# bwittmann/transoar

Hardware: AMD Instinct MI355X
Metric: training-step CT volumes/s, 160x160x256 Focused-Decoder (higher is better)
Workload: dtype bf16

## Files before the change

### include/transoar_conv3d.h

```cpp
#ifndef TRANSOAR_CONV3D_H
#define TRANSOAR_CONV3D_H

#include <stddef.h>
#include <stdint.h>

#ifdef __cplusplus
extern "C" {
#endif

enum {
  TRANSOAR_CONV_OK = 0,
  TRANSOAR_CONV_ERR_NULL = -1,
  TRANSOAR_CONV_ERR_DIM = -2,
  TRANSOAR_CONV_ERR_CHANNELS = -3
};

int transoar_conv3d_k3_forward(const void* x, const void* wk, const float* bias, void* y,
                               int N, int D, int H, int W, int Cin, int Cout, int stride,
                               int dilated_input, void* hip_stream);

int transoar_conv3d_k3_wgrad(const void* gyT, const void* xT3, float* dw, int N, int D, int H,
                             int W, int Cin, int Do, int Ho, int Wo, int Cout, int stride_dh,
                             void* hip_stream);

int transoar_conv3d_k3_forward_c1(const void* x, const void* wk, const float* bias, void* y, int N, int D, int H,
                                  int W, int Cout, void* hip_stream);

int transoar_conv3d_k3_stat_rows(int N, int D, int H, int W, int Cin, int Cout, int stride);
int transoar_conv3d_k3_forward_stats(const void* x, const void* wk, const float* bias, void* y, float* stat_part,
                                     int N, int D, int H, int W, int Cin, int Cout, void* hip_stream);

int transoar_conv3d_c1_forward(const void* x, const float* w, void* y, int N, int D, int H,
                               int W, int Cout, void* hip_stream);

int transoar_conv3d_k3_wgrad_lds(const void* x, const void* dy, float* partial, int n_wg, int N, int D,
                                 int H, int W, int Cin, int Cout, int ci0, int ci_n, int co0, int co_n,
                                 void* hip_stream);
int transoar_conv3d_k3_wgrad_tr(const void* x, const void* dy, float* partial, int n_wg, int N, int D,
                                 int H, int W, int Cin, int Cout, int ci0, int ci_n, int co0, int co_n,
                                 void* hip_stream);

int transoar_conv3d_c1_wgrad(const void* x, const void* dy, float* partial, int n_partial, int N, int D,
                             int H, int W, int Cout, void* hip_stream);
int transoar_conv3d_c1_wgrad_tr(const void* x, const void* dy, float* partial, int n_partial, int N, int D,
                                int H, int W, int Cout, void* hip_stream);

int transoar_layout_bf16(const void* in, void* out, int N, long V, int C, int to_channels_first,
                         void* hip_stream);

int transoar_conv3d_abi_version(void);

#ifdef __cplusplus
}
#endif
#endif
```

### include/transoar_instnorm.h

```cpp
#ifndef TRANSOAR_INSTNORM_H
#define TRANSOAR_INSTNORM_H

#ifdef __cplusplus
extern "C" {
#endif

enum {
  TRANSOAR_IN_OK = 0,
  TRANSOAR_IN_ERR_NULL = -1,
  TRANSOAR_IN_ERR_DIM = -2,
  TRANSOAR_IN_ERR_CHANNELS = -3
};

int transoar_instnorm_relu_forward(const void* x, const float* gamma, const float* beta, void* y,
                                   double* stats_ws, float* mean_rstd, int N, long V, int C,
                                   float eps, int relu, void* hip_stream);

int transoar_instnorm_relu_forward_parts(const void* x, const float* gamma, const float* beta, void* y,
                                         const float* stat_part, int rows_per_sample, double* stats_ws,
                                         float* mean_rstd, int N, long V, int C, float eps, int relu,
                                         void* hip_stream);

int transoar_instnorm_relu_backward(const void* x, const void* dy, const float* gamma,
                                    const float* beta, const float* mean_rstd, void* dx,
                                    double* red_ws, float* dparams, int N, long V, int C, int relu,
                                    void* hip_stream);

int transoar_instnorm_abi_version(void);

#ifdef __cplusplus
}
#endif
#endif
```

### transoar_amd/backbone.py

```python
import os

import torch
from torch import nn

from . import instnorm
from .conv3d import Conv3dK3, to_ncdhw
from .position_encoding import PositionEmbeddingLearned3D, PositionEmbeddingSine3D
from .swin_encoder import ConvPatchMerging, EncoderSwinBlock, PatchMerging
from .refine_block import DecoderDefAttnBlock
from .token_linear import token_linear


class EncoderCnnBlock(nn.Module):

    def __init__(self, in_channels, out_channels, kernel_size, stride, padding=1, bias=False,
                 affine=True, eps=1e-05):
        super().__init__()
        kernel_size, stride = tuple(kernel_size), tuple(stride)
        self._block = nn.Sequential(
            Conv3dK3(in_channels, out_channels, kernel_size, stride=stride, padding=padding, bias=bias),
            nn.InstanceNorm3d(out_channels, affine=affine, eps=eps),
            nn.ReLU(inplace=True),
            Conv3dK3(out_channels, out_channels, kernel_size, stride=1, padding=padding, bias=bias),
            nn.InstanceNorm3d(out_channels, affine=affine, eps=eps),
            nn.ReLU(inplace=True),
        )
        self._affine = affine

    fused_norm = True

    def _norm_relu(self, x, norm, part=None):
        if (EncoderCnnBlock.fused_norm and self._affine and x.dtype == torch.bfloat16
                and instnorm.supported(x, norm.num_features)):
            return instnorm.instance_norm_relu(x, norm.weight, norm.bias, norm.eps, relu=True, part=part)
        return torch.relu_(norm(x))

    def _conv_norm_relu(self, conv, norm, x):
        if (EncoderCnnBlock.fused_norm and self._affine and isinstance(conv, Conv3dK3) and norm.num_features <= 32):
            y, part = conv.forward_with_stats(x)
            if part is not None and not (y.dtype == torch.bfloat16 and instnorm.supported(y, norm.num_features)):
                part = None
            return self._norm_relu(y, norm, part)
        return self._norm_relu(conv(x), norm)

    def forward(self, x):
        if not x.is_cuda:
            return self._block(x)
        blk = self._block
        x = self._conv_norm_relu(blk[0], blk[1], x)
        return self._conv_norm_relu(blk[3], blk[4], x)


class Encoder(nn.Module):
    def __init__(self, config, debug=False):
        super().__init__()
        self._debug = debug
        self._stages = nn.ModuleList()
        cin, cout = config["in_channels"], config["start_channels"]
        swin = bool(config["use_encoder_attn"])
        depths = list(config["depths"])
        dpr = [float(v) for v in torch.linspace(0, config["drop_path_rate"], sum(depths))]
        merge = ConvPatchMerging if config["conv_merging"] else PatchMerging
        for stage_id, (kernel, stride) in enumerate(zip(config["conv_kernels"], config["strides"])):
            if swin and stage_id > 1:
                k = stage_id - 2
                stage = EncoderSwinBlock(
                    dim=cin, depth=depths[k], num_heads=config["num_heads"][k], window_size=config["window_size"],
                    mlp_ratio=config["mlp_ratio"], qkv_bias=config["qkv_bias"], qk_scale=config["qk_scale"],
                    drop=config["drop_rate"], attn_drop=config["attn_drop_rate"],
                    drop_path=dpr[sum(depths[:k]):sum(depths[:k + 1])], downsample=merge)
            else:
                stage = EncoderCnnBlock(cin, cout, kernel, stride)
            self._stages.append(stage)
            cin, cout = cout, cout * 2

    def forward(self, x):
        outputs = {}
        for i, stage in enumerate(self._stages):
            x = stage(x)
            outputs["C%d" % i] = x
        if self._debug:
            print("AttnFPN encoder shapes:", {k: list(v.shape) for k, v in outputs.items()})
            self._debug = False
        return outputs


def _gemm_conv_ok(f):
    return (f.is_cuda and f.dtype == torch.bfloat16 and f.dim() == 5 and f.shape[1] % 8 == 0
            and f.is_contiguous(memory_format=torch.channels_last_3d)
            and torch.is_autocast_enabled() and torch.get_autocast_gpu_dtype() == torch.bfloat16)
# ... 116 lines not shown
```

### transoar_amd/conv3d.py

```python
import ctypes
import os

import torch
import torch.nn.functional as F
from torch import nn

from . import _native
from . import rows as _rows
from . import conv_gemm as _cg

_PKG = os.path.dirname(os.path.abspath(__file__))
_LIB_PATH = os.path.join(_PKG, "libtransoar_conv3d.so")
ABI_VERSION = 5


def _load():
    if not os.path.exists(_LIB_PATH):
        raise _native.NativeLibraryError("%s is not built (python transoar_amd/_build.py)" % _LIB_PATH)
    lib = ctypes.CDLL(_LIB_PATH)
    i, p = ctypes.c_int, ctypes.c_void_p
    lib.transoar_conv3d_k3_forward.restype = i
    lib.transoar_conv3d_k3_forward.argtypes = [p, p, p, p] + [i] * 8 + [p]
    lib.transoar_conv3d_k3_wgrad.restype = i
    lib.transoar_conv3d_k3_wgrad.argtypes = [p, p, p] + [i] * 10 + [p]
    lib.transoar_conv3d_k3_wgrad_lds.restype = i
    lib.transoar_conv3d_k3_wgrad_lds.argtypes = [p, p, p, i] + [i] * 10 + [p]
    lib.transoar_conv3d_k3_wgrad_tr.restype = i
    lib.transoar_conv3d_k3_wgrad_tr.argtypes = [p, p, p, i] + [i] * 10 + [p]
    lib.transoar_conv3d_c1_wgrad.restype = i
    lib.transoar_conv3d_c1_wgrad.argtypes = [p, p, p, i] + [i] * 5 + [p]
    lib.transoar_conv3d_c1_wgrad_tr.restype = i
    lib.transoar_conv3d_c1_wgrad_tr.argtypes = [p, p, p, i] + [i] * 5 + [p]
    lib.transoar_conv3d_k3_stat_rows.restype = i
    lib.transoar_conv3d_k3_stat_rows.argtypes = [i] * 7
    lib.transoar_conv3d_k3_forward_stats.restype = i
    lib.transoar_conv3d_k3_forward_stats.argtypes = [p, p, p, p, p] + [i] * 6 + [p]
    lib.transoar_conv3d_k3_forward_c1.restype = i
    lib.transoar_conv3d_k3_forward_c1.argtypes = [p, p, p, p] + [i] * 5 + [p]
    lib.transoar_conv3d_c1_forward.restype = i
    lib.transoar_conv3d_c1_forward.argtypes = [p, p, p] + [i] * 5 + [p]
    lib.transoar_layout_bf16.restype = i
    lib.transoar_layout_bf16.argtypes = [p, p, i, ctypes.c_long, i, i, p]
    lib.transoar_conv3d_abi_version.restype = i
    if lib.transoar_conv3d_abi_version() != ABI_VERSION:
        raise _native.NativeLibraryError("%s: ABI mismatch, rebuild" % _LIB_PATH)
    return lib


lib = _load()
CL3D = torch.channels_last_3d


def _check(rc, what):
    if rc != 0:
        raise RuntimeError("%s failed with code %d" % (what, rc))


def _stream():
    return torch.cuda.current_stream().cuda_stream


class _Relayout(torch.autograd.Function):

    @staticmethod
    def forward(ctx, t, to_channels_first):
        return _relayout_raw(t, to_channels_first)

    @staticmethod
    def backward(ctx, g):
        return g, None


def _relayout(t, to_channels_first):
    if t.requires_grad and torch.is_grad_enabled():
        return _Relayout.apply(t, to_channels_first)
    return _relayout_raw(t, to_channels_first)


def _relayout_raw(t, to_channels_first):
    n, c = t.shape[:2]
    v = t.shape[2] * t.shape[3] * t.shape[4]
    out = torch.empty(t.shape, dtype=t.dtype, device=t.device,
                      memory_format=torch.contiguous_format if to_channels_first else CL3D)
    with torch.cuda.device(t.device):
        _check(lib.transoar_layout_bf16(t.data_ptr(), out.data_ptr(), n, v, c, 1 if to_channels_first else 0,
# ... 59 lines not shown
        return None
    if ci == 1:
        y = torch.empty((n, d, h, w, co), dtype=torch.bfloat16, device=x.device).permute(0, 4, 1, 2, 3)
    else:
        y = torch.empty((n, co, d, h, w), dtype=torch.bfloat16, device=x.device, memory_format=CL3D)
    part = torch.empty((rows, 2, 32), dtype=torch.float32, device=x.device)
    with torch.cuda.device(x.device):
        _check(lib.transoar_conv3d_k3_forward_stats(x.data_ptr(), wk.data_ptr(), bias.data_ptr() if bias is not None else None,
                                                    y.data_ptr(), part.data_ptr(), n, d, h, w, ci, co, _stream()),
               "transoar_conv3d_k3_forward_stats")
    return y, part


def wgrad_operands(x, gy, stride):
    ow = gy.shape[4]
    gy_t = gy.permute(1, 0, 2, 3, 4).contiguous()
    x_t = F.pad(x.permute(1, 0, 2, 3, 4).contiguous(), (1, 1))
    x_t3 = torch.stack([x_t[..., kw: kw + stride * (ow - 1) + 1: stride] for kw in range(3)])
    return x_t3, gy_t


def conv3d_k3_wgrad(x, gy, stride):
    n, ci, d, h, w = x.shape
    co, od, oh, ow = gy.shape[1], gy.shape[2], gy.shape[3], gy.shape[4]
    x_t3, gy_t = wgrad_operands(x, gy, stride)
    cin_p = (ci + 7) // 8 * 8
    dw = torch.zeros((27, co, cin_p), dtype=torch.float32, device=x.device)
    with torch.cuda.device(x.device):
        _check(lib.transoar_conv3d_k3_wgrad(gy_t.data_ptr(), x_t3.data_ptr(), dw.data_ptr(), n, d, h, ow, ci,
                                            od, oh, ow, co, stride, _stream()), "transoar_conv3d_k3_wgrad")
    return dw[:, :, :ci].view(3, 3, 3, co, ci).permute(3, 4, 0, 1, 2)


C1_WGRAD_PARTIALS = 3200
C1_WGRAD_TR = os.environ.get("TRANSOAR_C1_WGRAD_TR", "1") != "0"
C1_WGRAD_TR_PARTIALS = 1024


def _colsum(partial):
    flat = partial.view(partial.shape[0], -1)
    return _rows.colsum_small(flat) if _rows.colsum_small_usable(flat) else flat.sum(0)


def conv3d_c1_wgrad(x, gy):
    n, _, d, h, w = x.shape
    co = gy.shape[1]
    tr = C1_WGRAD_TR and co % 8 == 0 and w % 64 == 0 and w <= 256
    n_part = min(C1_WGRAD_TR_PARTIALS, n * d * h) if tr else min(C1_WGRAD_PARTIALS, max(1, (n * d * h + 3) // 4))
    partial = torch.empty((n_part, 32, 32), dtype=torch.float32, device=x.device)
    with torch.cuda.device(x.device):
        fn = lib.transoar_conv3d_c1_wgrad_tr if tr else lib.transoar_conv3d_c1_wgrad
        _check(fn(x.data_ptr(), gy.data_ptr(), partial.data_ptr(), n_part, n, d, h, w, co, _stream()), "transoar_conv3d_c1_wgrad")
    return _colsum(partial).view(32, 32)[:co, :27].reshape(co, 1, 3, 3, 3)


LDS_WGRAD_GROUPS = 512
LDS_WGRAD_TR = os.environ.get("TRANSOAR_WGRAD_TR", "1") != "0"
LDS_WGRAD_TR_GROUPS = 512


def conv3d_k3_wgrad_lds(x, gy):
    n, ci, d, h, w = x.shape
    co = gy.shape[1]
    dw = torch.empty((co, ci, 27), dtype=torch.float32, device=x.device)
    for co0 in range(0, co, 32):
        for ci0 in range(0, ci, 32):
            co_n, ci_n = min(32, co - co0), min(32, ci - ci0)
            groups = LDS_WGRAD_TR_GROUPS if LDS_WGRAD_TR else LDS_WGRAD_GROUPS
            fn = lib.transoar_conv3d_k3_wgrad_tr if LDS_WGRAD_TR else lib.transoar_conv3d_k3_wgrad_lds
            partial = torch.empty((groups, 27, 32, 32), dtype=torch.float32, device=x.device)
            with torch.cuda.device(x.device):
                _check(fn(x.data_ptr(), gy.data_ptr(), partial.data_ptr(), groups, n, d, h, w, ci, co, ci0, ci_n, co0, co_n, _stream()),
                       "transoar_conv3d_k3_wgrad_lds")
            dw[co0:co0 + co_n, ci0:ci0 + ci_n] = _colsum(partial).view(27, 32, 32)[:, :co_n, :ci_n].permute(1, 2, 0)
    return dw.view(co, ci, 3, 3, 3)


def lds_wgrad_supported(x, gy):
    ci, co = x.shape[1], gy.shape[1]
    return (ci % 8 == 0 and co % 8 == 0 and ci <= 64 and co <= 64 and x.shape[-1] % 64 == 0
            and x.is_contiguous(memory_format=CL3D) and gy.is_contiguous(memory_format=CL3D))


def c1_wgrad_supported(x, gy):
    return x.shape[1] == 1 and gy.shape[1] <= 32 and x.shape[-1] % 16 == 0 and x.is_contiguous()


class _Conv3dK3(torch.autograd.Function):
    @staticmethod
    def forward(ctx, x, weight, bias, stride, packs=None, want_stats=False):
        xb = x.to(torch.bfloat16).contiguous() if x.shape[1] == 1 else _as_ndhwc(x)
        ci = xb.shape[1]
        wkt = None
        if want_stats:
            res = None
            if stride == 1 and (ci == 1 or not _use_gemm(ci, weight.shape[0], stride)):
                wk = _pack_taps(F.pad(weight, (0, 0, 0, 0, 0, 0, 0, 7)) if ci == 1 else weight)
                res = conv3d_k3_forward_stats(xb, wk, bias.float() if bias is not None else None)
            if res is not None:
                ctx.save_for_backward(xb, weight, None)
                ctx.stride, ctx.has_bias, ctx.two = stride, bias is not None, True
                ctx.mark_non_differentiable(res[1])
                return res
        ctx.two = want_stats
        if ci == 1:
            n, _, d, h, w = xb.shape
# ... 96 lines not shown
```

### transoar_amd/csrc/conv3d.hip

```cpp
#include <hip/hip_runtime.h>
#include <algorithm>
#include <cstdlib>
#include <stdint.h>

#include "../../include/transoar_conv3d.h"

namespace transoar {

using bf16x8 = __attribute__((ext_vector_type(8))) __bf16;
using f32x16 = __attribute__((ext_vector_type(16))) float;
using u32x4c = __attribute__((ext_vector_type(4))) unsigned int;
using u32x2c = __attribute__((ext_vector_type(2))) unsigned int;

__device__ __forceinline__ unsigned short f2bf(float f) {
  return __builtin_bit_cast(unsigned short, static_cast<__bf16>(f));
}
__device__ __forceinline__ unsigned pack2_bf16(float a, float b) {
  typedef float f32x2_t __attribute__((ext_vector_type(2)));
  typedef __bf16 bf16x2_t __attribute__((ext_vector_type(2)));
  return __builtin_bit_cast(unsigned, __builtin_convertvector(f32x2_t{a, b}, bf16x2_t));
}
__device__ __forceinline__ float bf2f(unsigned short b) {
  return __uint_as_float(static_cast<unsigned int>(b) << 16);
}
// ... 168 lines not shown
  __shared__ __attribute__((aligned(16))) unsigned char halo[kLtHaloVox * VP];
  const int lane = threadIdx.x & 63;
  const int wave = threadIdx.x >> 6;
  const int col = lane & 31, half = lane >> 5;

  const long per = (n_tiles + 7) >> 3;
  const long trow = static_cast<long>(blockIdx.x & 7) * per + (blockIdx.x >> 3);
  if (trow >= n_tiles || (blockIdx.x >> 3) >= per) return;
  const int th = static_cast<int>(trow % tiles_h);
  const long t2 = trow / tiles_h;
  const int td = static_cast<int>(t2 % tiles_d);
  const int n = static_cast<int>(t2 / tiles_d);
  const int d0 = td * kLtD, h0 = th * kLtH;

  const __amdgpu_buffer_rsrc_t xr =
      __builtin_amdgcn_make_buffer_rsrc(const_cast<unsigned short*>(x), 0, static_cast<int>(x_bytes), 0x00020000);
  const __amdgpu_buffer_rsrc_t wr =
      __builtin_amdgcn_make_buffer_rsrc(const_cast<unsigned short*>(wk), 0, static_cast<int>(w_bytes), 0x00020000);

  constexpr int PIECES = kLtHaloVox * CPT;
  constexpr int ROUNDS = (PIECES + 255) / 256;
  u32x4c stage[ROUNDS];
  auto fetch = [&](int w0) {
#pragma unroll
    for (int r = 0; r < ROUNDS; ++r) {
      const int p = r * 256 + static_cast<int>(threadIdx.x);
      const int hv = p / CPT, c = p - hv * CPT;
      const int row = hv / (kLtW + 2), wi = hv - row * (kLtW + 2);
      const int hd = row / (kLtH + 2), hh = row - hd * (kLtH + 2);
      const int d = d0 - 1 + hd, h = h0 - 1 + hh, w = w0 - 1 + wi;
      const bool ok = p < PIECES && static_cast<unsigned>(d) < static_cast<unsigned>(g.D) &&
                      static_cast<unsigned>(h) < static_cast<unsigned>(g.H) && static_cast<unsigned>(w) < static_cast<unsigned>(g.W);
      if constexpr (C1) {
        const unsigned off = ok ? static_cast<unsigned>(((n * g.D + d) * g.H + h) * g.W + w) * 2u : kOOB;
        const unsigned short v = __builtin_amdgcn_raw_buffer_load_b16(xr, off, 0, 0);
        stage[r] = u32x4c{static_cast<unsigned>(v), 0u, 0u, 0u};
      } else {
        const unsigned off = ok ? (static_cast<unsigned>(((n * g.D + d) * g.H + h) * g.W + w) * CPT + c) * 16u : kOOB;
        stage[r] = __builtin_amdgcn_raw_buffer_load_b128(xr, off, 0, 0);
      }
    }
  };
  float srun[4] = {0.f, 0.f, 0.f, 0.f};
  fetch(0);
  for (int tw = 0; tw < tiles_w; ++tw) {
  const int w0 = tw * kLtW;
#pragma unroll
  for (int r = 0; r < ROUNDS; ++r) {
    const int p = r * 256 + static_cast<int>(threadIdx.x);
    if (p < PIECES) *reinterpret_cast<u32x4c*>(halo + p * 16) = stage[r];
  }
  __syncthreads();
  if (tw + 1 < tiles_w) fetch(w0 + kLtW);

  f32x16 acc[MT];
#pragma unroll
  for (int t = 0; t < MT; ++t)
#pragma unroll
    for (int r = 0; r < 16; ++r) acc[t][r] = 0.f;

  constexpr int n_chunks = 9 * CPT;
  constexpr int n_steps = (n_chunks + 1) / 2;
  const unsigned char* lane_base = halo + ((wave * (kLtH + 2)) * (kLtW + 2) + col) * VP;
  const unsigned w_lane = static_cast<unsigned>(col) * g.CinP * 2u;
  const bool co_ok = col < g.Cout;
  const unsigned w_tap = static_cast<unsigned>(g.Cout) * g.CinP * 2u;
  if constexpr (CPT == 3 && !C1) {
    auto load_w = [&](auto gc, int kd, bf16x8 (&wf)[3]) {
      constexpr int gi = decltype(gc)::value;
      constexpr int kw0 = gi < 3 ? gi : (gi == 3 ? 0 : 2), kw1 = gi < 3 ? gi : (gi == 3 ? 1 : 2);
      constexpr int c80 = gi < 3 ? 0 : 2, c81 = gi < 3 ? 1 : 2;
      const bool ok = co_ok && (half ? gi != 4 : true);
      const unsigned base = kd * 9 * w_tap + w_lane + (half ? kw1 * w_tap + c81 * 16 : kw0 * w_tap + c80 * 16);
#pragma unroll
      for (int kh = 0; kh < 3; ++kh)
        wf[kh] = __builtin_bit_cast(bf16x8, __builtin_amdgcn_raw_buffer_load_b128(wr, ok ? base + kh * 3 * w_tap : kOOB, 0, 0));
    };
    bf16x8 wcur[3];
    load_w(ConvIntC<0>{}, 0, wcur);
#pragma unroll 1
    for (int kd = 0; kd < 3; ++kd) {
      const unsigned char* plane = lane_base + kd * (kLtH + 2) * (kLtW + 2) * VP;
      static_for_conv<0, 5>([&](auto gc) {
        constexpr int gi = decltype(gc)::value;
        constexpr int kw0 = gi < 3 ? gi : (gi == 3 ? 0 : 2), kw1 = gi < 3 ? gi : (gi == 3 ? 1 : 2);
        constexpr int c80 = gi < 3 ? 0 : 2, c81 = gi < 3 ? 1 : 2;
        bf16x8 wnext[3];
        if constexpr (gi + 1 < 5) load_w(ConvIntC<gi + 1>{}, kd, wnext);
        else load_w(ConvIntC<0>{}, kd + 1, wnext);
        const unsigned char* src = plane + (half ? kw1 * VP + c81 * 16 : kw0 * VP + c80 * 16);
        bf16x8 xr[MT + 2];
#pragma unroll
        for (int r = 0; r < MT + 2; ++r) xr[r] = __builtin_bit_cast(bf16x8, *reinterpret_cast<const u32x4c*>(src + r * (kLtW + 2) * VP));
#pragma unroll
        for (int kh = 0; kh < 3; ++kh)
#pragma unroll
          for (int t = 0; t < MT; ++t) acc[t] = __builtin_amdgcn_mfma_f32_32x32x16_bf16(wcur[kh], xr[t + kh], acc[t], 0, 0, 0);
#pragma unroll
        for (int kh = 0; kh < 3; ++kh) wcur[kh] = wnext[kh];
      });
    }
  } else {
#pragma unroll 1
  for (int kd = 0; kd < 3; ++kd) {
    const unsigned char* plane = lane_base + kd * (kLtH + 2) * (kLtW + 2) * VP;
    const unsigned w_plane = kd * 9 * w_tap + w_lane;
    auto weight_fragment = [&](auto sc) {
// ... 292 lines not shown
  f32x16 acc;
#pragma unroll
  for (int r = 0; r < 16; ++r) acc[r] = 0.f;

  const long row0 = (static_cast<long>(blockIdx.x) * 4 + wave) * rows_per_wave;
  for (int rr = 0; rr < rows_per_wave; ++rr) {
    const long row = row0 + rr;
    if (row >= n_rows) break;
    const int h = static_cast<int>(row % H);
    const long bd = row / H;
    const int d = static_cast<int>(bd % D);
    const int id = d + kd, ih = h + kh;
    const bool row_ok = tap_ok && static_cast<unsigned>(id) < static_cast<unsigned>(D) &&
                        static_cast<unsigned>(ih) < static_cast<unsigned>(H);
    const unsigned short* xrow = x + ((bd - d + (row_ok ? id : d)) * H + (row_ok ? ih : h)) * W;
    const unsigned short* dyrow = dy + row * W * Cout + (co_ok ? col : 0);
    for (int w0 = 0; w0 < W; w0 += 16) {
      unsigned short av[8], bv[8];
#pragma unroll
      for (int j = 0; j < 8; ++j) {
        const int w = w0 + 8 * kg + j;
        av[j] = dyrow[static_cast<long>(w) * Cout];
        const int iw = w + kw;
        const unsigned short xv = xrow[min(max(iw, 0), W - 1)];
        bv[j] = (row_ok && static_cast<unsigned>(iw) < static_cast<unsigned>(W)) ? xv : static_cast<unsigned short>(0);
      }
      u32x4c ap, bp;
#pragma unroll
      for (int j = 0; j < 4; ++j) {
        ap[j] = co_ok ? (static_cast<unsigned>(av[2 * j]) | (static_cast<unsigned>(av[2 * j + 1]) << 16)) : 0u;
        bp[j] = static_cast<unsigned>(bv[2 * j]) | (static_cast<unsigned>(bv[2 * j + 1]) << 16);
      }
      acc = __builtin_amdgcn_mfma_f32_32x32x16_bf16(__builtin_bit_cast(bf16x8, ap), __builtin_bit_cast(bf16x8, bp), acc,
                                                    0, 0, 0);
    }
  }
#pragma unroll
  for (int r = 0; r < 16; ++r) red[wave][r][lane] = acc[r];
  __syncthreads();
  if (wave == 0) {
    float* out = partial + static_cast<long>(blockIdx.x) * 1024;
#pragma unroll
    for (int r = 0; r < 16; ++r) {
      const float v = red[0][r][lane] + red[1][r][lane] + red[2][r][lane] + red[3][r][lane];
      out[((r & 3) + 8 * (r >> 2) + 4 * kg) * 32 + col] = v;
    }
  }
}

typedef short c1_s16x4 __attribute__((ext_vector_type(4)));
typedef short c1_s16x8 __attribute__((ext_vector_type(8)));
constexpr int kC1XP = 256 + 16;

template <int CO8>
__global__ __launch_bounds__(256) void conv3d_c1_wgrad_tr(const unsigned short* __restrict__ x, const unsigned short* __restrict__ dy,
                                                          float* __restrict__ partial, int N, int D, int H, int W, int Cout,
                                                          long n_rows, int rows_per_wg, unsigned x_bytes, unsigned dy_bytes) {
  __shared__ __attribute__((aligned(16))) unsigned char dyt[256 * 64 + 512];
  __shared__ __attribute__((aligned(16))) unsigned short xs[3][10][kC1XP];
  const int tid = threadIdx.x, lane = tid & 63, wave = tid >> 6;
  const int kg = lane >> 5;
  const __amdgpu_buffer_rsrc_t rx = __builtin_amdgcn_make_buffer_rsrc(const_cast<unsigned short*>(x), 0, static_cast<int>(x_bytes), 0x00020000);
  const __amdgpu_buffer_rsrc_t rdy = __builtin_amdgcn_make_buffer_rsrc(const_cast<unsigned short*>(dy), 0, static_cast<int>(dy_bytes), 0x00020000);
  for (int i = tid; i < (256 * 64 + 512) / 4; i += 256) reinterpret_cast<unsigned*>(dyt)[i] = 0u;
  for (int i = tid; i < 3 * 10 * kC1XP / 2; i += 256) reinterpret_cast<unsigned*>(&xs[0][0][0])[i] = 0u;

  f32x16 acc;
#pragma unroll
  for (int r = 0; r < 16; ++r) acc[r] = 0.f;
  const int t_row = 8 * kg + ((lane & 15) >> 2), t_ch = 16 * ((lane >> 4) & 1) + 4 * (lane & 3);
  const unsigned char* a_base = dyt + (64 * wave + t_row) * 64 + t_ch * 2;
  const int tap = lane & 31;
  const unsigned short* b_base = tap < 27 ? &xs[tap % 3][tap / 3][64 * wave + 8 * kg] : &xs[0][9][64 * wave + 8 * kg];
  typedef __attribute__((address_space(3))) c1_s16x4 lds_s16x4;

  const long row_beg = static_cast<long>(blockIdx.x) * rows_per_wg, row_end = min(n_rows, row_beg + rows_per_wg);
  u32x4c pdy[CO8], px[2];
  const int dy_pieces = W * CO8;
  auto prefetch = [&](long row) {
#pragma unroll
    for (int k = 0; k < CO8; ++k) {
      const int p = tid + 256 * k;
      pdy[k] = __builtin_amdgcn_raw_buffer_load_b128(rdy, p < dy_pieces ? static_cast<unsigned>(row) * static_cast<unsigned>(dy_pieces * 16) + p * 16 : 0x80000000u, 0, 0);
    }
    const int h = static_cast<int>(row % H);
    const long bd = row / H;
    const int d = static_cast<int>(bd % D);
#pragma unroll
    for (int k = 0; k < 2; ++k) {
      const int i = tid + 256 * k, r = i >> 5, piece = i & 31;
      const int id = d + r / 3 - 1, ih = h + r % 3 - 1;
      const bool ok = r < 9 && piece * 8 < W && static_cast<unsigned>(id) < static_cast<unsigned>(D) && static_cast<unsigned>(ih) < static_cast<unsigned>(H);
      px[k] = __builtin_amdgcn_raw_buffer_load_b128(rx, ok ? static_cast<unsigned>(((bd - d + id) * H + ih) * W + piece * 8) * 2u : 0x80000000u, 0, 0);
    }
  };
  if (row_beg < row_end) prefetch(row_beg);
  __syncthreads();
  for (long row = row_beg; row < row_end; ++row) {
#pragma unroll
    for (int k = 0; k < CO8; ++k) {
      const int p = tid + 256 * k;
      if (p < dy_pieces) *reinterpret_cast<u32x4c*>(dyt + (p / CO8) * 64 + (p % CO8) * 16) = pdy[k];
    }
#pragma unroll
    for (int k = 0; k < 2; ++k) {
      const int i = tid + 256 * k, r = i >> 5, piece = i & 31;
      const u32x4c v = px[k];
      unsigned left = __shfl_up(v[3], 1), right = __shfl_down(v[0], 1);
      if (piece == 0) left = 0u;
      if (piece * 8 + 8 >= W) right = 0u;
      if (r < 9 && piece * 8 < W) {
        u32x4c lo, hi;
        lo[0] = __builtin_amdgcn_alignbit(v[0], left, 16); lo[1] = __builtin_amdgcn_alignbit(v[1], v[0], 16);
        lo[2] = __builtin_amdgcn_alignbit(v[2], v[1], 16); lo[3] = __builtin_amdgcn_alignbit(v[3], v[2], 16);
        hi[0] = __builtin_amdgcn_alignbit(v[1], v[0], 16); hi[1] = __builtin_amdgcn_alignbit(v[2], v[1], 16);
        hi[2] = __builtin_amdgcn_alignbit(v[3], v[2], 16); hi[3] = __builtin_amdgcn_alignbit(right, v[3], 16);
        *reinterpret_cast<u32x4c*>(&xs[0][r][piece * 8]) = lo;
        *reinterpret_cast<u32x4c*>(&xs[1][r][piece * 8]) = v;
        *reinterpret_cast<u32x4c*>(&xs[2][r][piece * 8]) = hi;
      }
    }
    __syncthreads();
    if (row + 1 < row_end) prefetch(row + 1);
    if (64 * wave < W) {
#pragma unroll
      for (int ks = 0; ks < 4; ++ks) {
        const c1_s16x4 alo = __builtin_amdgcn_ds_read_tr16_b64_v4i16((lds_s16x4*)(a_base + ks * 16 * 64));
        const c1_s16x4 ahi = __builtin_amdgcn_ds_read_tr16_b64_v4i16((lds_s16x4*)(a_base + ks * 16 * 64 + 4 * 64));
        const c1_s16x8 a = __builtin_shufflevector(alo, ahi, 0, 1, 2, 3, 4, 5, 6, 7);
        const c1_s16x8 b = *reinterpret_cast<const c1_s16x8*>(b_base + ks * 16);
        acc = __builtin_amdgcn_mfma_f32_32x32x16_bf16(__builtin_bit_cast(bf16x8, a), __builtin_bit_cast(bf16x8, b), acc, 0, 0, 0);
      }
    }
    __syncthreads();
  }
  float* red = reinterpret_cast<float*>(dyt);
#pragma unroll
  for (int r = 0; r < 16; ++r) red[(wave * 16 + r) * 64 + lane] = acc[r];
  __syncthreads();
  if (wave == 0) {
    float* out = partial + static_cast<long>(blockIdx.x) * 1024;
#pragma unroll
    for (int r = 0; r < 16; ++r) {
      const int co = (r & 3) + 8 * (r >> 2) + 4 * kg;
      const float v = red[r * 64 + lane] + red[(16 + r) * 64 + lane] + red[(32 + r) * 64 + lane] + red[(48 + r) * 64 + lane];
      out[co * 32 + tap] = (co < Cout && tap < 27) ? v : 0.f;
    }
  }
}

#include "conv3d_wgrad_lds.hpp"
#include "conv3d_wgrad_tr.hpp"

__global__ __launch_bounds__(256) void layout_vc_to_cv(const unsigned short* __restrict__ in,
                                                        unsigned short* __restrict__ out, long V, int C) {
// ... 213 lines not shown
  hipStream_t st = static_cast<hipStream_t>(hip_stream);
  auto xs = static_cast<const unsigned short*>(x);
  auto ds = static_cast<const unsigned short*>(dy);
#define TRANSOAR_WT_CASE(CI, CO)                                                                         \
  if (ci_n == 8 * CI && co_n == 8 * CO) {                                                                \
    hipLaunchKernelGGL((conv3d_k3_wgrad_tr<CI, CO>), dim3(static_cast<unsigned>(n_wg)), dim3(kWtThreads), 0, st, xs, ds, \
                       partial, N, D, H, W, h_chunks, h_chunk, Cin, ci0, Cout, co0);                  \
    return static_cast<int>(hipGetLastError());                                                          \
  }
  TRANSOAR_WT_CASE(1, 1) TRANSOAR_WT_CASE(1, 2) TRANSOAR_WT_CASE(1, 3) TRANSOAR_WT_CASE(1, 4)
  TRANSOAR_WT_CASE(2, 1) TRANSOAR_WT_CASE(2, 2) TRANSOAR_WT_CASE(2, 3) TRANSOAR_WT_CASE(2, 4)
  TRANSOAR_WT_CASE(3, 1) TRANSOAR_WT_CASE(3, 2) TRANSOAR_WT_CASE(3, 3) TRANSOAR_WT_CASE(3, 4)
  TRANSOAR_WT_CASE(4, 1) TRANSOAR_WT_CASE(4, 2) TRANSOAR_WT_CASE(4, 3) TRANSOAR_WT_CASE(4, 4)
#undef TRANSOAR_WT_CASE
  return TRANSOAR_CONV_ERR_CHANNELS;
}

extern "C" int transoar_conv3d_c1_wgrad(const void* x, const void* dy, float* partial, int n_partial, int N, int D, int H,
                                        int W, int Cout, void* hip_stream) {
  if (!x || !dy || !partial) return TRANSOAR_CONV_ERR_NULL;
  if (N <= 0 || D <= 0 || H <= 0 || W <= 0 || Cout <= 0 || n_partial <= 0) return TRANSOAR_CONV_ERR_DIM;
  if (Cout > 32 || (W & 15)) return TRANSOAR_CONV_ERR_CHANNELS;
  const long n_rows = static_cast<long>(N) * D * H;
  const int rows_per_wave = static_cast<int>((n_rows + static_cast<long>(n_partial) * 4 - 1) / (static_cast<long>(n_partial) * 4));
  hipLaunchKernelGGL(conv3d_c1_wgrad, dim3(static_cast<unsigned>(n_partial)), dim3(256), 0,
                     static_cast<hipStream_t>(hip_stream), static_cast<const unsigned short*>(x),
                     static_cast<const unsigned short*>(dy), partial, N, D, H, W, Cout, n_rows, rows_per_wave);
  return static_cast<int>(hipGetLastError());
}

extern "C" int transoar_conv3d_c1_wgrad_tr(const void* x, const void* dy, float* partial, int n_partial, int N, int D, int H,
                                           int W, int Cout, void* hip_stream) {
  if (!x || !dy || !partial) return TRANSOAR_CONV_ERR_NULL;
  if (N <= 0 || D <= 0 || H <= 0 || W <= 0 || Cout <= 0 || n_partial <= 0) return TRANSOAR_CONV_ERR_DIM;
  if (Cout > 32 || (Cout & 7) || (W & 63) || W > 256) return TRANSOAR_CONV_ERR_CHANNELS;
  const long n_rows = static_cast<long>(N) * D * H;
  const long xb = n_rows * W * 2, dyb = n_rows * W * Cout * 2;
  if (dyb >= 0x7ffffff0L) return TRANSOAR_CONV_ERR_DIM;
  const int rows_per_wg = static_cast<int>((n_rows + n_partial - 1) / n_partial);
#define TRANSOAR_C1TR(CO8)                                                                                                          \
  hipLaunchKernelGGL(conv3d_c1_wgrad_tr<CO8>, dim3(static_cast<unsigned>(n_partial)), dim3(256), 0, static_cast<hipStream_t>(hip_stream), \
                     static_cast<const unsigned short*>(x), static_cast<const unsigned short*>(dy), partial, N, D, H, W, Cout, n_rows,   \
                     rows_per_wg, static_cast<unsigned>(xb), static_cast<unsigned>(dyb))
  switch (Cout / 8) {
    case 1: TRANSOAR_C1TR(1); break;
    case 2: TRANSOAR_C1TR(2); break;
    case 3: TRANSOAR_C1TR(3); break;
    default: TRANSOAR_C1TR(4); break;
  }
#undef TRANSOAR_C1TR
  return static_cast<int>(hipGetLastError());
}

extern "C" int transoar_conv3d_c1_forward(const void* x, const float* w, void* y, int N, int D, int H, int W,
                                          int Cout, void* hip_stream) {
  if (!x || !w || !y) return TRANSOAR_CONV_ERR_NULL;
  if (N <= 0 || D <= 0 || H <= 0 || W <= 0 || Cout <= 0) return TRANSOAR_CONV_ERR_DIM;
  if ((Cout & 7) || Cout > transoar::kC1MaxCout) return TRANSOAR_CONV_ERR_CHANNELS;
  const long n_vox = static_cast<long>(N) * D * H * W;
  hipLaunchKernelGGL(conv3d_c1_fwd, dim3(static_cast<unsigned>((n_vox + 255) / 256)), dim3(256), 0,
                     static_cast<hipStream_t>(hip_stream), static_cast<const unsigned short*>(x), w,
                     static_cast<unsigned short*>(y), N, D, H, W, Cout, n_vox);
  return static_cast<int>(hipGetLastError());
}

extern "C" int transoar_layout_bf16(const void* in, void* out, int N, long V, int C, int to_channels_first,
                                    void* hip_stream) {
  if (!in || !out) return TRANSOAR_CONV_ERR_NULL;
  if (N <= 0 || V <= 0 || C <= 0) return TRANSOAR_CONV_ERR_DIM;
  if (C & 7) return TRANSOAR_CONV_ERR_CHANNELS;
  const dim3 grid(static_cast<unsigned>((V + 255) / 256), static_cast<unsigned>(N));
  hipStream_t st = static_cast<hipStream_t>(hip_stream);
  if (to_channels_first)
    hipLaunchKernelGGL(layout_vc_to_cv, grid, dim3(256), 0, st, static_cast<const unsigned short*>(in),
                       static_cast<unsigned short*>(out), V, C);
  else
    hipLaunchKernelGGL(layout_cv_to_vc, grid, dim3(256), 0, st, static_cast<const unsigned short*>(in),
                       static_cast<unsigned short*>(out), V, C);
  return static_cast<int>(hipGetLastError());
}

extern "C" int transoar_conv3d_abi_version(void) { return 5; }
```

### transoar_amd/csrc/instnorm.hip

```cpp
#include <hip/hip_runtime.h>
#include <stdint.h>

#include "../../include/transoar_instnorm.h"

namespace transoar {

using u32x4n = __attribute__((ext_vector_type(4))) unsigned int;
constexpr int kINThreads = 192;
constexpr int kINDepth = 4;
constexpr int kINBlocksPerCU = 4;
constexpr int kINDepthDx = 2;

__device__ __forceinline__ void unpack8(const u32x4n& r, float (&o)[8]) {
#pragma unroll
  for (int i = 0; i < 4; ++i) {
    o[2 * i] = __uint_as_float(r[i] << 16);
    o[2 * i + 1] = __uint_as_float(r[i] & 0xffff0000u);
  }
}
__device__ __forceinline__ unsigned short f2bf_n(float f) {
  return __builtin_bit_cast(unsigned short, static_cast<__bf16>(f));
}
__device__ __forceinline__ unsigned pack2_bf16_n(float a, float b) {
  typedef float f32x2_t __attribute__((ext_vector_type(2)));
// ... 261 lines not shown
  const int rc = check(x, y, N, V, C);
  if (rc) return rc;
  if (!gamma || !beta || !stats_ws || !mean_rstd) return TRANSOAR_IN_ERR_NULL;
  hipStream_t st = static_cast<hipStream_t>(hip_stream);
  const int bps = pick_blocks(V, N, C);
  hipError_t e = hipMemsetAsync(stats_ws, 0, sizeof(double) * 2 * N * C, st);
  if (e != hipSuccess) return static_cast<int>(e);
  hipLaunchKernelGGL(instnorm_stats, dim3(N * bps), dim3(kINThreads), 0, st, static_cast<const unsigned short*>(x),
                     stats_ws, V, C, bps);
  hipLaunchKernelGGL(instnorm_apply_relu, dim3(N * bps), dim3(kINThreads), 0, st,
                     static_cast<const unsigned short*>(x), stats_ws, gamma, beta, static_cast<unsigned short*>(y),
                     mean_rstd, V, C, eps, bps, relu);
  return static_cast<int>(hipGetLastError());
}

extern "C" int transoar_instnorm_relu_forward_parts(const void* x, const float* gamma, const float* beta, void* y,
                                                    const float* stat_part, int rows_per_sample, double* stats_ws,
                                                    float* mean_rstd, int N, long V, int C, float eps, int relu,
                                                    void* hip_stream) {
  const int rc = check(x, y, N, V, C);
  if (rc) return rc;
  if (!gamma || !beta || !stats_ws || !mean_rstd || !stat_part) return TRANSOAR_IN_ERR_NULL;
  if (C > 32 || rows_per_sample <= 0) return TRANSOAR_IN_ERR_DIM;
  hipStream_t st = static_cast<hipStream_t>(hip_stream);
  const int bps = pick_blocks(V, N, C);
  hipError_t e = hipMemsetAsync(stats_ws, 0, sizeof(double) * 2 * N * C, st);
  if (e != hipSuccess) return static_cast<int>(e);
  hipLaunchKernelGGL(instnorm_stats_from_parts, dim3(N, kPartBlocks), dim3(256), 0, st, stat_part, rows_per_sample, C, stats_ws);
  hipLaunchKernelGGL(instnorm_apply_relu, dim3(N * bps), dim3(kINThreads), 0, st,
                     static_cast<const unsigned short*>(x), stats_ws, gamma, beta, static_cast<unsigned short*>(y),
                     mean_rstd, V, C, eps, bps, relu);
  return static_cast<int>(hipGetLastError());
}

extern "C" int transoar_instnorm_relu_backward(const void* x, const void* dy, const float* gamma, const float* beta,
                                               const float* mean_rstd, void* dx, double* red_ws, float* dparams, int N, long V,
                                               int C, int relu, void* hip_stream) {
  const int rc = check(x, dy, N, V, C);
  if (rc) return rc;
  if (!gamma || !beta || !mean_rstd || !dx || !red_ws) return TRANSOAR_IN_ERR_NULL;
  hipStream_t st = static_cast<hipStream_t>(hip_stream);
  const int bps = pick_blocks(V, N, C);
  hipError_t e = hipMemsetAsync(red_ws, 0, sizeof(double) * 2 * N * C, st);
  if (e != hipSuccess) return static_cast<int>(e);
  hipLaunchKernelGGL(instnorm_bwd_reduce, dim3(N * bps), dim3(kINThreads), 0, st,
                     static_cast<const unsigned short*>(x), static_cast<const unsigned short*>(dy), mean_rstd, gamma,
                     beta, red_ws, V, C, bps, relu);
  hipLaunchKernelGGL(instnorm_bwd_dx, dim3(N * bps), dim3(kINThreads), 0, st, static_cast<const unsigned short*>(x),
                     static_cast<const unsigned short*>(dy), mean_rstd, gamma, beta, red_ws,
                     static_cast<unsigned short*>(dx), V, C, bps, relu, dparams, N);
  return static_cast<int>(hipGetLastError());
}

extern "C" int transoar_instnorm_abi_version(void) { return 3; }
```

### transoar_amd/instnorm.py

```python
import ctypes
import os

import torch

from . import _native
from .conv3d import to_ndhwc

_PKG = os.path.dirname(os.path.abspath(__file__))
_LIB_PATH = os.path.join(_PKG, "libtransoar_instnorm.so")


def _load():
    if not os.path.exists(_LIB_PATH):
        raise _native.NativeLibraryError("%s is not built (python transoar_amd/_build.py)" % _LIB_PATH)
    lib = ctypes.CDLL(_LIB_PATH)
    i, p, lg, f = ctypes.c_int, ctypes.c_void_p, ctypes.c_long, ctypes.c_float
    lib.transoar_instnorm_relu_forward.restype = i
    lib.transoar_instnorm_relu_forward.argtypes = [p, p, p, p, p, p, i, lg, i, f, i, p]
    lib.transoar_instnorm_relu_forward_parts.restype = i
    lib.transoar_instnorm_relu_forward_parts.argtypes = [p, p, p, p, p, i, p, p, i, lg, i, f, i, p]
    lib.transoar_instnorm_relu_backward.restype = i
    lib.transoar_instnorm_relu_backward.argtypes = [p, p, p, p, p, p, p, p, i, lg, i, i, p]
    lib.transoar_instnorm_abi_version.restype = i
    if lib.transoar_instnorm_abi_version() != 3:
        raise _native.NativeLibraryError("%s: ABI mismatch, rebuild" % _LIB_PATH)
    return lib


lib = _load()
CL3D = torch.channels_last_3d


def supported(x, channels):
    return (x.is_cuda and x.dtype == torch.bfloat16 and x.dim() == 5 and channels % 8 == 0
            and 192 % (channels // 8) == 0)


class _InstNormReLU(torch.autograd.Function):
    @staticmethod
    def forward(ctx, x, gamma, beta, eps, relu, part=None):
        x = to_ndhwc(x)
        n, c = x.shape[:2]
        v = x.shape[2] * x.shape[3] * x.shape[4]
        y = torch.empty_like(x, memory_format=CL3D)
        g32, b32 = gamma.float().contiguous(), beta.float().contiguous()
        ws = torch.empty((n, c, 2), dtype=torch.float64, device=x.device)
        mean_rstd = torch.empty((n, c, 2), dtype=torch.float32, device=x.device)
        with torch.cuda.device(x.device):
            if part is not None:
                rc = lib.transoar_instnorm_relu_forward_parts(x.data_ptr(), g32.data_ptr(), b32.data_ptr(), y.data_ptr(),
                                                              part.data_ptr(), part.shape[0] // n, ws.data_ptr(), mean_rstd.data_ptr(),
                                                              n, v, c, float(eps), 1 if relu else 0,
                                                              torch.cuda.current_stream().cuda_stream)
            else:
                rc = lib.transoar_instnorm_relu_forward(x.data_ptr(), g32.data_ptr(), b32.data_ptr(), y.data_ptr(),
                                                        ws.data_ptr(), mean_rstd.data_ptr(), n, v, c, float(eps),
                                                        1 if relu else 0, torch.cuda.current_stream().cuda_stream)
        if rc != 0:
            raise RuntimeError("transoar_instnorm_relu_forward failed with code %d" % rc)
        ctx.save_for_backward(x, g32, b32, mean_rstd)
        ctx.relu, ctx.param_dtype = relu, gamma.dtype
        return y

    @staticmethod
    def backward(ctx, dy):
        x, g32, b32, mean_rstd = ctx.saved_tensors
        dy = to_ndhwc(dy)
        n, c = x.shape[:2]
        v = x.shape[2] * x.shape[3] * x.shape[4]
        dx = torch.empty_like(x, memory_format=CL3D)
        red = torch.empty((n, c, 2), dtype=torch.float64, device=x.device)
        with torch.cuda.device(x.device):
            dparams = torch.empty((2, c), dtype=torch.float32, device=x.device)
            rc = lib.transoar_instnorm_relu_backward(x.data_ptr(), dy.data_ptr(), g32.data_ptr(), b32.data_ptr(),
                                                     mean_rstd.data_ptr(), dx.data_ptr(), red.data_ptr(), dparams.data_ptr(), n, v, c,
                                                     1 if ctx.relu else 0, torch.cuda.current_stream().cuda_stream)
        if rc != 0:
            raise RuntimeError("transoar_instnorm_relu_backward failed with code %d" % rc)
        return dx, dparams[1].to(ctx.param_dtype), dparams[0].to(ctx.param_dtype), None, None, None


def instance_norm_relu(x, gamma, beta, eps=1e-5, relu=True, part=None):
    return _InstNormReLU.apply(x, gamma, beta, eps, relu, part)
```

Measured before the change: 64.42.

## Fuse stem conv instance-norm backward dx into c1 weight-gradient kernel

```diff
diff --git a/include/transoar_conv3d.h b/include/transoar_conv3d.h
--- a/include/transoar_conv3d.h
+++ b/include/transoar_conv3d.h
@@ -44,6 +44,10 @@
                              int H, int W, int Cout, void* hip_stream);
 int transoar_conv3d_c1_wgrad_tr(const void* x, const void* dy, float* partial, int n_partial, int N, int D,
                                 int H, int W, int Cout, void* hip_stream);
+int transoar_conv3d_c1_wgrad_tr_norm(const void* x, const void* dy, const void* xn, const float* mean_rstd,
+                                     const float* gamma, const float* beta, const double* red, float* dparams,
+                                     float* partial, int n_partial, int N, int D, int H, int W, int Cout, int relu,
+                                     void* hip_stream);
 
 int transoar_layout_bf16(const void* in, void* out, int N, long V, int C, int to_channels_first,
                          void* hip_stream);
diff --git a/include/transoar_instnorm.h b/include/transoar_instnorm.h
--- a/include/transoar_instnorm.h
+++ b/include/transoar_instnorm.h
@@ -26,6 +26,10 @@
                                     double* red_ws, float* dparams, int N, long V, int C, int relu,
                                     void* hip_stream);
 
+int transoar_instnorm_relu_backward_reduce(const void* x, const void* dy, const float* gamma,
+                                           const float* beta, const float* mean_rstd, double* red_ws,
+                                           int N, long V, int C, int relu, void* hip_stream);
+
 int transoar_instnorm_abi_version(void);
 
 #ifdef __cplusplus
diff --git a/transoar_amd/backbone.py b/transoar_amd/backbone.py
--- a/transoar_amd/backbone.py
+++ b/transoar_amd/backbone.py
@@ -35,7 +35,22 @@
             return instnorm.instance_norm_relu(x, norm.weight, norm.bias, norm.eps, relu=True, part=part)
         return torch.relu_(norm(x))
 
+    stem_norm_bwd = os.environ.get("TRANSOAR_STEM_NORM_BWD", "1") != "0"
+
+    def _stem(self, conv, norm, x):
+        if not (EncoderCnnBlock.stem_norm_bwd and EncoderCnnBlock.fused_norm and self._affine and isinstance(conv, Conv3dK3)
+                and conv.in_channels == 1 and Conv3dK3.enabled and Conv3dK3.stats_in_epilogue):
+            return None
+        amp = torch.is_autocast_enabled() and x.is_cuda and torch.get_autocast_gpu_dtype() == torch.bfloat16
+        xb = x.to(torch.bfloat16) if (amp and x.dtype != torch.bfloat16) else x
+        if not instnorm.stem_supported(xb, conv, norm):
+            return None
+        return instnorm.stem_conv_norm_relu(xb, conv, norm)
+
     def _conv_norm_relu(self, conv, norm, x):
+        y = self._stem(conv, norm, x)
+        if y is not None:
+            return y
         if (EncoderCnnBlock.fused_norm and self._affine and isinstance(conv, Conv3dK3) and norm.num_features <= 32):
             y, part = conv.forward_with_stats(x)
             if part is not None and not (y.dtype == torch.bfloat16 and instnorm.supported(y, norm.num_features)):
diff --git a/transoar_amd/conv3d.py b/transoar_amd/conv3d.py
--- a/transoar_amd/conv3d.py
+++ b/transoar_amd/conv3d.py
@@ -11,7 +11,7 @@
 
 _PKG = os.path.dirname(os.path.abspath(__file__))
 _LIB_PATH = os.path.join(_PKG, "libtransoar_conv3d.so")
-ABI_VERSION = 5
+ABI_VERSION = 6
 
 
 def _load():
@@ -31,6 +31,8 @@
     lib.transoar_conv3d_c1_wgrad.argtypes = [p, p, p, i] + [i] * 5 + [p]
     lib.transoar_conv3d_c1_wgrad_tr.restype = i
     lib.transoar_conv3d_c1_wgrad_tr.argtypes = [p, p, p, i] + [i] * 5 + [p]
+    lib.transoar_conv3d_c1_wgrad_tr_norm.restype = i
+    lib.transoar_conv3d_c1_wgrad_tr_norm.argtypes = [p] * 9 + [i] * 7 + [p]
     lib.transoar_conv3d_k3_stat_rows.restype = i
     lib.transoar_conv3d_k3_stat_rows.argtypes = [i] * 7
     lib.transoar_conv3d_k3_forward_stats.restype = i
@@ -196,6 +198,25 @@
         fn = lib.transoar_conv3d_c1_wgrad_tr if tr else lib.transoar_conv3d_c1_wgrad
         _check(fn(x.data_ptr(), gy.data_ptr(), partial.data_ptr(), n_part, n, d, h, w, co, _stream()), "transoar_conv3d_c1_wgrad")
     return _colsum(partial).view(32, 32)[:co, :27].reshape(co, 1, 3, 3, 3)
+
+
+def c1_wgrad_norm_supported(x, co):
+    n, ci, d, h, w = x.shape
+    return (C1_WGRAD_TR and ci == 1 and co % 8 == 0 and co <= 32 and w % 64 == 0 and w <= 256
+            and n * d * h * w * co * 2 < 0x7ffffff0)
+
+
+def conv3d_c1_wgrad_norm(x, gy, xn, mean_rstd, gamma, beta, red, relu=True):
+    n, _, d, h, w = x.shape
+    co = gy.shape[1]
+    n_part = min(C1_WGRAD_TR_PARTIALS, n * d * h)
+    partial = torch.empty((n_part, 32, 32), dtype=torch.float32, device=x.device)
+    dparams = torch.empty((2, co), dtype=torch.float32, device=x.device)
+    with torch.cuda.device(x.device):
+        _check(lib.transoar_conv3d_c1_wgrad_tr_norm(x.data_ptr(), gy.data_ptr(), xn.data_ptr(), mean_rstd.data_ptr(), gamma.data_ptr(),
+                                                    beta.data_ptr(), red.data_ptr(), dparams.data_ptr(), partial.data_ptr(), n_part,
+                                                    n, d, h, w, co, 1 if relu else 0, _stream()), "transoar_conv3d_c1_wgrad_tr_norm")
+    return _colsum(partial).view(32, 32)[:co, :27].reshape(co, 1, 3, 3, 3), dparams
 
 
 LDS_WGRAD_GROUPS = 512
diff --git a/transoar_amd/csrc/conv3d.hip b/transoar_amd/csrc/conv3d.hip
--- a/transoar_amd/csrc/conv3d.hip
+++ b/transoar_amd/csrc/conv3d.hip
@@ -244,7 +244,6 @@
   }
   __syncthreads();
   if (tw + 1 < tiles_w) fetch(w0 + kLtW);
-
   f32x16 acc[MT];
 #pragma unroll
   for (int t = 0; t < MT; ++t)
@@ -643,16 +642,60 @@
 typedef short c1_s16x8 __attribute__((ext_vector_type(8)));
 constexpr int kC1XP = 256 + 16;
 
-template <int CO8>
-__global__ __launch_bounds__(256) void conv3d_c1_wgrad_tr(const unsigned short* __restrict__ x, const unsigned short* __restrict__ dy,
+struct C1NormArgs {
+  const unsigned short* xn;
+  const float* mean_rstd;
+  const float* gamma;
+  const float* beta;
+  const double* red;
+  float* dparams;
+  int relu;
+};
+
+__device__ __forceinline__ u32x4c c1_norm_dx(const u32x4c& pxn, const u32x4c& pg, const float (*nc)[8], int c0, int relu) {
+  typedef float c1_f32x4 __attribute__((ext_vector_type(4)));
+  u32x4c r;
+#pragma unroll
+  for (int i = 0; i < 4; ++i) {
+    float o[2];
+#pragma unroll
+    for (int j = 0; j < 2; ++j) {
+      const float f = j ? __uint_as_float(pxn[i] & 0xffff0000u) : __uint_as_float(pxn[i] << 16);
+      const float g = j ? __uint_as_float(pg[i] & 0xffff0000u) : __uint_as_float(pg[i] << 16);
+      const c1_f32x4 a = *reinterpret_cast<const c1_f32x4*>(&nc[c0 + 2 * i + j][0]);
+      const c1_f32x4 b = *reinterpret_cast<const c1_f32x4*>(&nc[c0 + 2 * i + j][4]);
+      const float xh = (f - a[0]) * a[1];
+      const float gg = (!relu || xh * a[2] + a[3] > 0.f) ? g : 0.f;
+      o[j] = a[1] * a[2] * (gg - b[0] - xh * b[1]);
+    }
+    r[i] = pack2_bf16(o[0], o[1]);
+  }
+  return r;
+}
+
+template <int CO8, bool NORM = false>
+__global__ __launch_bounds__(256, NORM ? 4 : 1) void conv3d_c1_wgrad_tr(const unsigned short* __restrict__ x, const unsigned short* __restrict__ dy,
                                                           float* __restrict__ partial, int N, int D, int H, int W, int Cout,
-                                                          long n_rows, int rows_per_wg, unsigned x_bytes, unsigned dy_bytes) {
+                                                          long n_rows, int rows_per_wg, unsigned x_bytes, unsigned dy_bytes,
+                                                          C1NormArgs na = C1NormArgs{}) {
   __shared__ __attribute__((aligned(16))) unsigned char dyt[256 * 64 + 512];
   __shared__ __attribute__((aligned(16))) unsigned short xs[3][10][kC1XP];
+  __shared__ __attribute__((aligned(16))) float nc[NORM ? 32 : 1][8];
   const int tid = threadIdx.x, lane = tid & 63, wave = tid >> 6;
   const int kg = lane >> 5;
   const __amdgpu_buffer_rsrc_t rx = __builtin_amdgcn_make_buffer_rsrc(const_cast<unsigned short*>(x), 0, static_cast<int>(x_bytes), 0x00020000);
   const __amdgpu_buffer_rsrc_t rdy = __builtin_amdgcn_make_buffer_rsrc(const_cast<unsigned short*>(dy), 0, static_cast<int>(dy_bytes), 0x00020000);
+  const __amdgpu_buffer_rsrc_t rxn = __builtin_amdgcn_make_buffer_rsrc(const_cast<unsigned short*>(NORM ? na.xn : dy), 0, static_cast<int>(dy_bytes), 0x00020000);
+  if constexpr (NORM) {
+    if (na.dparams && blockIdx.x == 0) {
+      for (int i = tid; i < 2 * Cout; i += 256) {
+        const int k = i / Cout, c = i - k * Cout;
+        double s = 0.0;
+        for (int nn = 0; nn < N; ++nn) s += na.red[(static_cast<long>(nn) * Cout + c) * 2 + k];
+        na.dparams[i] = static_cast<float>(s);
+      }
+    }
+  }
   for (int i = tid; i < (256 * 64 + 512) / 4; i += 256) reinterpret_cast<unsigned*>(dyt)[i] = 0u;
   for (int i = tid; i < 3 * 10 * kC1XP / 2; i += 256) reinterpret_cast<unsigned*>(&xs[0][0][0])[i] = 0u;
 
@@ -666,13 +709,15 @@
   typedef __attribute__((address_space(3))) c1_s16x4 lds_s16x4;
 
   const long row_beg = static_cast<long>(blockIdx.x) * rows_per_wg, row_end = min(n_rows, row_beg + rows_per_wg);
-  u32x4c pdy[CO8], px[2];
+  u32x4c pdy[CO8], px[2], pxn[NORM ? CO8 : 1];
   const int dy_pieces = W * CO8;
   auto prefetch = [&](long row) {
 #pragma unroll
     for (int k = 0; k < CO8; ++k) {
       const int p = tid + 256 * k;
-      pdy[k] = __builtin_amdgcn_raw_buffer_load_b128(rdy, p < dy_pieces ? static_cast<unsigned>(row) * static_cast<unsigned>(dy_pieces * 16) + p * 16 : 0x80000000u, 0, 0);
+      const unsigned off = p < dy_pieces ? static_cast<unsigned>(row) * static_cast<unsigned>(dy_pieces * 16) + p * 16 : 0x80000000u;
+      pdy[k] = __builtin_amdgcn_raw_buffer_load_b128(rdy, off, 0, 0);
+      if constexpr (NORM) pxn[k] = __builtin_amdgcn_raw_buffer_load_b128(rxn, off, 0, 0);
     }
     const int h = static_cast<int>(row % H);
     const long bd = row / H;
@@ -687,11 +732,33 @@
   };
   if (row_beg < row_end) prefetch(row_beg);
   __syncthreads();
+  long cur_n = -1;
   for (long row = row_beg; row < row_end; ++row) {
+    if constexpr (NORM) {
+      const long ns = row / (static_cast<long>(D) * H);
+      if (ns != cur_n) {
+        if (tid < Cout) {
+          const long k = ns * Cout + tid;
+          const double V = static_cast<double>(D) * H * W;
+          nc[tid][0] = na.mean_rstd[k * 2];
+          nc[tid][1] = na.mean_rstd[k * 2 + 1];
+          nc[tid][2] = na.gamma[tid];
+          nc[tid][3] = na.beta[tid];
+          nc[tid][4] = static_cast<float>(na.red[k * 2] / V);
+          nc[tid][5] = static_cast<float>(na.red[k * 2 + 1] / V);
+        }
+        cur_n = ns;
+        __syncthreads();
+      }
+    }
 #pragma unroll
     for (int k = 0; k < CO8; ++k) {
       const int p = tid + 256 * k;
-      if (p < dy_pieces) *reinterpret_cast<u32x4c*>(dyt + (p / CO8) * 64 + (p % CO8) * 16) = pdy[k];
+      if (p < dy_pieces) {
+        u32x4c v = pdy[k];
+        if constexpr (NORM) v = c1_norm_dx(pxn[k], v, nc, (p % CO8) * 8, na.relu);
+        *reinterpret_cast<u32x4c*>(dyt + (p / CO8) * 64 + (p % CO8) * 16) = v;
+      }
     }
 #pragma unroll
     for (int k = 0; k < 2; ++k) {
@@ -1011,6 +1078,34 @@
   return static_cast<int>(hipGetLastError());
 }
 
+extern "C" int transoar_conv3d_c1_wgrad_tr_norm(const void* x, const void* dy, const void* xn, const float* mean_rstd,
+                                                const float* gamma, const float* beta, const double* red, float* dparams,
+                                                float* partial, int n_partial, int N, int D, int H, int W, int Cout, int relu,
+                                                void* hip_stream) {
+  if (!x || !dy || !partial || !xn || !mean_rstd || !gamma || !beta || !red) return TRANSOAR_CONV_ERR_NULL;
+  if (N <= 0 || D <= 0 || H <= 0 || W <= 0 || Cout <= 0 || n_partial <= 0) return TRANSOAR_CONV_ERR_DIM;
+  if (Cout > 32 || (Cout & 7) || (W & 63) || W > 256) return TRANSOAR_CONV_ERR_CHANNELS;
+  const long n_rows = static_cast<long>(N) * D * H;
+  const long xb = n_rows * W * 2, dyb = n_rows * W * Cout * 2;
+  if (dyb >= 0x7ffffff0L) return TRANSOAR_CONV_ERR_DIM;
+  const int rows_per_wg = static_cast<int>((n_rows + n_partial - 1) / n_partial);
+  C1NormArgs na;
+  na.xn = static_cast<const unsigned short*>(xn);
+  na.mean_rstd = mean_rstd; na.gamma = gamma; na.beta = beta; na.red = red; na.dparams = dparams; na.relu = relu;
+#define TRANSOAR_C1TRN(CO8)                                                                                                                  \
+  hipLaunchKernelGGL((conv3d_c1_wgrad_tr<CO8, true>), dim3(static_cast<unsigned>(n_partial)), dim3(256), 0, static_cast<hipStream_t>(hip_stream), \
+                     static_cast<const unsigned short*>(x), static_cast<const unsigned short*>(dy), partial, N, D, H, W, Cout, n_rows,       \
+                     rows_per_wg, static_cast<unsigned>(xb), static_cast<unsigned>(dyb), na)
+  switch (Cout / 8) {
+    case 1: TRANSOAR_C1TRN(1); break;
+    case 2: TRANSOAR_C1TRN(2); break;
+    case 3: TRANSOAR_C1TRN(3); break;
+    default: TRANSOAR_C1TRN(4); break;
+  }
+#undef TRANSOAR_C1TRN
+  return static_cast<int>(hipGetLastError());
+}
+
 extern "C" int transoar_conv3d_c1_forward(const void* x, const float* w, void* y, int N, int D, int H, int W,
                                           int Cout, void* hip_stream) {
   if (!x || !w || !y) return TRANSOAR_CONV_ERR_NULL;
@@ -1039,4 +1134,4 @@
   return static_cast<int>(hipGetLastError());
 }
 
-extern "C" int transoar_conv3d_abi_version(void) { return 5; }
+extern "C" int transoar_conv3d_abi_version(void) { return 6; }
diff --git a/transoar_amd/csrc/instnorm.hip b/transoar_amd/csrc/instnorm.hip
--- a/transoar_amd/csrc/instnorm.hip
+++ b/transoar_amd/csrc/instnorm.hip
@@ -337,4 +337,20 @@
   return static_cast<int>(hipGetLastError());
 }
 
-extern "C" int transoar_instnorm_abi_version(void) { return 3; }
+extern "C" int transoar_instnorm_relu_backward_reduce(const void* x, const void* dy, const float* gamma, const float* beta,
+                                                      const float* mean_rstd, double* red_ws, int N, long V, int C, int relu,
+                                                      void* hip_stream) {
+  const int rc = check(x, dy, N, V, C);
+  if (rc) return rc;
+  if (!gamma || !beta || !mean_rstd || !red_ws) return TRANSOAR_IN_ERR_NULL;
+  hipStream_t st = static_cast<hipStream_t>(hip_stream);
+  const int bps = pick_blocks(V, N, C);
+  hipError_t e = hipMemsetAsync(red_ws, 0, sizeof(double) * 2 * N * C, st);
+  if (e != hipSuccess) return static_cast<int>(e);
+  hipLaunchKernelGGL(instnorm_bwd_reduce, dim3(N * bps), dim3(kINThreads), 0, st,
+                     static_cast<const unsigned short*>(x), static_cast<const unsigned short*>(dy), mean_rstd, gamma,
+                     beta, red_ws, V, C, bps, relu);
+  return static_cast<int>(hipGetLastError());
+}
+
+extern "C" int transoar_instnorm_abi_version(void) { return 4; }
diff --git a/transoar_amd/instnorm.py b/transoar_amd/instnorm.py
--- a/transoar_amd/instnorm.py
+++ b/transoar_amd/instnorm.py
@@ -2,8 +2,10 @@
 import os
 
 import torch
+import torch.nn.functional as F
 
 from . import _native
+from . import conv3d as _conv
 from .conv3d import to_ndhwc
 
 _PKG = os.path.dirname(os.path.abspath(__file__))
@@ -21,8 +23,10 @@
     lib.transoar_instnorm_relu_forward_parts.argtypes = [p, p, p, p, p, i, p, p, i, lg, i, f, i, p]
     lib.transoar_instnorm_relu_backward.restype = i
     lib.transoar_instnorm_relu_backward.argtypes = [p, p, p, p, p, p, p, p, i, lg, i, i, p]
+    lib.transoar_instnorm_relu_backward_reduce.restype = i
+    lib.transoar_instnorm_relu_backward_reduce.argtypes = [p, p, p, p, p, p, i, lg, i, i, p]
     lib.transoar_instnorm_abi_version.restype = i
-    if lib.transoar_instnorm_abi_version() != 3:
+    if lib.transoar_instnorm_abi_version() != 4:
         raise _native.NativeLibraryError("%s: ABI mismatch, rebuild" % _LIB_PATH)
     return lib
 
@@ -80,5 +84,64 @@
         return dx, dparams[1].to(ctx.param_dtype), dparams[0].to(ctx.param_dtype), None, None, None
 
 
+def backward_reduce(x, dy, g32, b32, mean_rstd, relu=True):
+    n, c = x.shape[:2]
+    v = x.shape[2] * x.shape[3] * x.shape[4]
+    red = torch.empty((n, c, 2), dtype=torch.float64, device=x.device)
+    with torch.cuda.device(x.device):
+        rc = lib.transoar_instnorm_relu_backward_reduce(x.data_ptr(), dy.data_ptr(), g32.data_ptr(), b32.data_ptr(),
+                                                        mean_rstd.data_ptr(), red.data_ptr(), n, v, c, 1 if relu else 0,
+                                                        torch.cuda.current_stream().cuda_stream)
+    if rc != 0:
+        raise RuntimeError("transoar_instnorm_relu_backward_reduce failed with code %d" % rc)
+    return red
+
+
+class _StemConvNormReLU(torch.autograd.Function):
+
+    @staticmethod
+    def forward(ctx, x, weight, gamma, beta, eps):
+        xb = x.to(torch.bfloat16).contiguous()
+        wk = _conv._pack_taps(F.pad(weight, (0, 0, 0, 0, 0, 0, 0, 7)))
+        y, part = _conv.conv3d_k3_forward_stats(xb, wk, None)
+        n, c = y.shape[:2]
+        v = y.shape[2] * y.shape[3] * y.shape[4]
+        out = torch.empty_like(y, memory_format=CL3D)
+        g32, b32 = gamma.float().contiguous(), beta.float().contiguous()
+        ws = torch.empty((n, c, 2), dtype=torch.float64, device=x.device)
+        mean_rstd = torch.empty((n, c, 2), dtype=torch.float32, device=x.device)
+        with torch.cuda.device(x.device):
+            rc = lib.transoar_instnorm_relu_forward_parts(y.data_ptr(), g32.data_ptr(), b32.data_ptr(), out.data_ptr(),
+                                                          part.data_ptr(), part.shape[0] // n, ws.data_ptr(), mean_rstd.data_ptr(),
+                                                          n, v, c, float(eps), 1, torch.cuda.current_stream().cuda_stream)
+        if rc != 0:
+            raise RuntimeError("transoar_instnorm_relu_forward_parts failed with code %d" % rc)
+        ctx.save_for_backward(xb, y, g32, b32, mean_rstd)
+        ctx.weight_dtype, ctx.param_dtype = weight.dtype, gamma.dtype
+        return out
+
+    @staticmethod
+    def backward(ctx, dy):
+        xb, y, g32, b32, mean_rstd = ctx.saved_tensors
+        dy = to_ndhwc(dy)
+        red = backward_reduce(y, dy, g32, b32, mean_rstd, True)
+        gw, dparams = _conv.conv3d_c1_wgrad_norm(xb, dy, y, mean_rstd, g32, b32, red, True)
+        return None, gw.to(ctx.weight_dtype), dparams[1].to(ctx.param_dtype), dparams[0].to(ctx.param_dtype), None
+
+
+def stem_supported(x, conv, norm):
+    if not (x.is_cuda and x.dtype == torch.bfloat16 and x.dim() == 5 and not x.requires_grad and conv.in_channels == 1
+            and conv.bias is None and conv.stride == (1, 1, 1) and norm.affine and _conv.hip_conv_supported(x, conv)):
+        return False
+    n, _, d, h, w = x.shape
+    co = conv.out_channels
+    return (co == norm.num_features and _conv.c1_wgrad_norm_supported(x, co) and co % 8 == 0 and 192 % (co // 8) == 0
+            and _conv.lib.transoar_conv3d_k3_stat_rows(n, d, h, w, 1, co, 1) != 0)
+
+
+def stem_conv_norm_relu(x, conv, norm):
+    return _StemConvNormReLU.apply(x, conv.weight, norm.weight, norm.bias, norm.eps)
+
+
 def instance_norm_relu(x, gamma, beta, eps=1e-5, relu=True, part=None):
     return _InstNormReLU.apply(x, gamma, beta, eps, relu, part)
```

New measurement: 64.69 (median of 6 runs). About the same (+0.4%).
